# zacharie12/Hypernet-image-captioning

Hardware: AMD Instinct MI355X
Metric: training images/sec at 1/2/4/8 MI355X, Flickr30k GRU+hypernet bs=128 (higher is better)
Workload: dtype f32; 1 GPU; Flickr30k-shaped GRU+additive-attention decoder + hypernet (3 style domains), full training step (fwd, CE, bwd, clip 5.0, Adam); per_gpu_batch=128, global_batch=128, T=20, P=49, D=2048, F=200, E=200, H=200, V=9684, hypernet_params=144906720, parallelism=dp1, launch=eager, next_theta_in_adam_pass=True, next_precompute_beside_adam=True, spinup_steps=0, deterministic_gradients=True

## Files before the change

hypernet-image-captioning_amd/caphn/_lib.py:

```python
import ctypes as C
import os

import torch

_HERE = os.path.dirname(os.path.abspath(__file__))
LIB_PATH = os.environ.get("CAPHN_LIB_PATH") or os.path.join(_HERE, "libcaphn.so")
MAX_HEADS = 8

c_fp = C.c_void_p


class HyperDesc(C.Structure):
    _fields_ = [("he", C.c_int), ("n_heads", C.c_int),
                ("k", C.c_int * MAX_HEADS), ("w", C.c_int * MAX_HEADS),
                ("base_w0", c_fp), ("base_b0", c_fp), ("base_w2", c_fp), ("base_b2", c_fp),
                ("w1", c_fp * MAX_HEADS), ("b1", c_fp * MAX_HEADS),
                ("w2", c_fp * MAX_HEADS), ("b2", c_fp * MAX_HEADS),
                ("d_in", C.c_int), ("d_mid", C.c_int)]


class HyperGrads(C.Structure):
    _fields_ = [("g_base_w0", c_fp), ("g_base_b0", c_fp), ("g_base_w2", c_fp), ("g_base_b2", c_fp),
                ("g_w1", c_fp * MAX_HEADS), ("g_b1", c_fp * MAX_HEADS),
                ("g_w2", c_fp * MAX_HEADS), ("g_b2", c_fp * MAX_HEADS),
# ... 8 lines not shown

_DEC_FIELDS = ("fc0_w", "fc0_b", "fc2_w", "fc2_b", "embed_w", "out_w", "out_b", "Wa_w", "Wa_b",
               "Ua_w", "Ua_b", "va_w", "va_b", "inith_w", "inith_b", "w_ih", "w_hh", "b_ih", "b_hh",
               "initc_w", "initc_b") + tuple(f"{a}{i}" for a in ("lw_ih", "lw_hh", "lb_ih", "lb_hh") for i in range(3))


class DecoderParams(C.Structure):
    _fields_ = [(n, c_fp) for n in _DEC_FIELDS]


class DecoderGrads(C.Structure):
    _fields_ = [(n, c_fp) for n in _DEC_FIELDS]


class AdamHParams(C.Structure):
    _fields_ = [("lr", C.c_float), ("beta1", C.c_float), ("beta2", C.c_float), ("eps", C.c_float),
                ("step", C.c_int), ("dev_scalars", c_fp), ("zero_gfac", C.c_int)]


class RankJob(C.Structure):
    _fields_ = [("W", c_fp), ("m", c_fp), ("v", c_fp), ("gfac", c_fp), ("ldg", C.c_size_t), ("afac", c_fp), ("lda", C.c_size_t),
                ("next_a", c_fp), ("next_bias", c_fp), ("next_theta", c_fp), ("rows", C.c_int), ("k", C.c_int),
                ("next_pack", c_fp), ("pack_H", C.c_int), ("pack_HA", C.c_int), ("pack_pitch", C.c_int), ("pack_hrows", C.c_int)]


class PairPack(C.Structure):
    _fields_ = [("wp", c_fp), ("H", C.c_int), ("HA", C.c_int), ("pitch", C.c_int), ("hrows", C.c_int)]


MAX_LAYERS = 4


class PlainDims(C.Structure):
    _fields_ = [(n, C.c_int) for n in ("B", "T", "E", "H", "V", "L", "cell")]


class AttnDims(C.Structure):
    _fields_ = [(n, C.c_int) for n in ("bs", "nh", "dh", "tq", "tk", "q_ldt", "q_ldb", "k_ldt", "k_ldb", "v_ldt", "v_ldb",
                                       "o_ldt", "o_ldb")] + [("scale", C.c_float), ("dropout_p", C.c_float),
                                                             ("seed", C.c_uint64)]


class PlainParams(C.Structure):
    _fields_ = [("embed_w", c_fp), ("out_w", c_fp), ("out_b", c_fp),
                ("w_ih", c_fp * MAX_LAYERS), ("w_hh", c_fp * MAX_LAYERS), ("b_ih", c_fp * MAX_LAYERS), ("b_hh", c_fp * MAX_LAYERS)]


class PlainGrads(C.Structure):
    _fields_ = [("embed_w", c_fp), ("out_w", c_fp), ("out_b", c_fp),
                ("w_ih", c_fp * MAX_LAYERS), ("w_hh", c_fp * MAX_LAYERS), ("b_ih", c_fp * MAX_LAYERS), ("b_hh", c_fp * MAX_LAYERS),
                ("features", c_fp)]


class SearchCfg(C.Structure):
    _fields_ = [("n_images", C.c_int), ("beam", C.c_int), ("max_steps", C.c_int), ("zero_pad_rule", C.c_int),
                ("lookup_first", C.c_int), ("first_token", C.c_int64), ("end_token", C.c_int64)]


SIGNATURES = {
    "caphn_abi_version": (C.c_int, []),
    "caphn_device_arch": (C.c_int, [C.c_char_p, C.c_int]),
    "caphn_device_error": (C.c_int, [C.c_int]),
    "caphn_gemm_f32": (C.c_int, [C.c_int, C.c_int, C.c_int, C.c_int, C.c_int, c_fp, C.c_int, c_fp, C.c_int,
                                 c_fp, C.c_int, c_fp, c_fp, C.c_int, C.c_int, C.c_int, c_fp]),
    "caphn_split3_bf16": (C.c_int, [c_fp, C.c_int, C.c_int, C.c_int, c_fp, C.c_int, C.c_size_t, C.c_int, c_fp]),
    "caphn_gemm_planes_f32": (C.c_int, [C.c_int, C.c_int, C.c_int, C.c_int, C.c_int, c_fp, C.c_int, c_fp, C.c_int, C.c_size_t,
                                        c_fp, C.c_int, c_fp, C.c_int, C.c_size_t, c_fp, C.c_int, c_fp, c_fp, C.c_int, C.c_int,
                                        C.c_int, C.c_int, c_fp]),
    "caphn_zero_f32": (C.c_int, [c_fp, C.c_size_t, c_fp]),
    "caphn_lrelu_bwd_f32": (C.c_int, [C.c_size_t, c_fp, c_fp, c_fp, c_fp]),
    "caphn_axpy_f32": (C.c_int, [C.c_size_t, C.c_float, c_fp, c_fp, c_fp]),
    "caphn_scale_f32": (C.c_int, [C.c_size_t, c_fp, c_fp, c_fp, c_fp]),
    "caphn_add_dropout_f32": (C.c_int, [C.c_size_t, c_fp, c_fp, C.c_float, C.c_uint64, C.c_uint64, c_fp, c_fp]),
    "caphn_dropout_f32": (C.c_int, [C.c_size_t, C.c_float, C.c_uint64, C.c_uint64, c_fp, c_fp, c_fp]),
    "caphn_colsum_workspace_bytes": (C.c_size_t, [C.c_int, C.c_int]),
    "caphn_linear_wgrad_f32": (C.c_int, [C.c_int, C.c_int, C.c_int, c_fp, C.c_int, c_fp, C.c_int, c_fp, C.c_int, c_fp, c_fp, c_fp]),
    "caphn_colsum_f32": (C.c_int, [C.c_int, C.c_int, c_fp, C.c_int, c_fp, c_fp, c_fp]),
    "caphn_hyper_acts_floats": (C.c_int, [C.POINTER(HyperDesc)]),
    "caphn_hyper_forward": (C.c_int, [C.POINTER(HyperDesc), c_fp, c_fp, c_fp, c_fp]),
    "caphn_hyper_backward_workspace_bytes": (C.c_size_t, [C.POINTER(HyperDesc)]),
    "caphn_hyper_backward": (C.c_int, [C.POINTER(HyperDesc), c_fp, c_fp, C.POINTER(HyperGrads), c_fp, c_fp]),
    "caphn_decoder_workspace_bytes": (C.c_size_t, [C.POINTER(DecoderDims)]),
    "caphn_decoder_forward": (C.c_int, [C.POINTER(DecoderDims), C.POINTER(DecoderParams), c_fp, c_fp,
                                        c_fp, c_fp, c_fp, c_fp]),
    "caphn_decoder_pair_prep": (C.c_int, [C.POINTER(DecoderDims), C.POINTER(DecoderParams), c_fp, c_fp]),
    "caphn_decoder_pair_pack_desc": (C.c_int, [C.POINTER(DecoderDims), c_fp, C.POINTER(PairPack)]),
    "caphn_decoder_precompute": (C.c_int, [C.POINTER(DecoderDims), C.POINTER(DecoderParams), c_fp, c_fp, c_fp, c_fp]),
    "caphn_decoder_inputs": (C.c_int, [C.POINTER(DecoderDims), C.POINTER(DecoderParams), c_fp, c_fp, c_fp]),
    "caphn_decoder_lookup": (C.c_int, [C.POINTER(DecoderDims), C.POINTER(DecoderParams), c_fp, c_fp, c_fp]),
    "caphn_decoder_prepare_rows": (C.c_int, [C.POINTER(DecoderDims), c_fp, C.c_int64, c_fp, c_fp]),
    "caphn_decoder_forward_sampled": (C.c_int, [C.POINTER(DecoderDims), C.POINTER(DecoderParams), c_fp, c_fp,
# ... 123 lines not shown
```

hypernet-image-captioning_amd/csrc/decoder.hip:

```cpp
#include "common.h"
#include "decoder_internal.h"
#include "gemm_internal.h"
#include <algorithm>
#include <initializer_list>
#include <mutex>

int g_tune_deterministic = 0;
int g_tune_rec_pair = 1;
int g_tune_rec_rotate = 1;
int g_tune_vocab_order = 1;
int g_tune_branch_mask = 7;
int g_tune_splitk_target = 1280;
int g_tune_chain_main = 0;
int g_tune_hops = 0;
int g_tune_fork = 4;
int g_tune_join_chain = 0;
int g_tune_sk_dhs = 0, g_tune_sk_vocab_w = 0;
#define RUN(x) do { int _rc = (x); if (_rc != CAPHN_OK) return _rc; } while (0)

namespace {

struct Side {
    hipStream_t st[3];
    enum { D_FORK = 0, D_JOIN = 1, D_X = 4, D_MS = 10, D_PRE_F = 14, D_PRE_ALL = 15, D_COUNT = 16 };
    struct Dep { hipEvent_t ev; unsigned seq = 0; bool by_value = false; };
    Dep deps[D_COUNT];
    unsigned* vals = nullptr;
    unsigned counter = 0;
    bool values = false;
    bool pre_valid = false;
    const void* pre_ws = nullptr;
    bool ready = false, on = false;
    bool forked[3] = {false, false, false};
    hipStream_t main = nullptr;
    int init() {
        if (ready) return CAPHN_OK;
        static std::mutex mu;
        std::lock_guard<std::mutex> lock(mu);
        if (ready) return CAPHN_OK;
        for (auto& s : st) if (hipStreamCreateWithFlags(&s, hipStreamNonBlocking) != hipSuccess) return CAPHN_ELAUNCH;
// ... 626 lines not shown
    a.drop_p = d->dropout_p; a.drop_seed = d->dropout_seed;
    const int ang = w.L1 > 0 ? 0 : pair ? caphn_rec_pair_bwd_groups(P, H) : caphn_rec_bwd_groups(P, H);
    if (ang > 0) { a.dWaf = ws + w.dWaf; a.apart = ws + w.apart; }
    if (w.L1 > 0) {
        RUN(caphn_zero_f32(ws + w.dcarry, (size_t)B * H, s));
        a.dHs = ws + w.dH0; a.dh0 = ws + w.dcarry; a.drop_p = 0.f;
        for (int t = T - 1; t >= 0; --t) {
            RUN(layers_backward(d, p, w, ws, t + 1, ws + w.dHs + (size_t)t * H, T * H, ws + w.dcarry, ws + w.dH0 + (size_t)t * H, T * H, s));
            a.t0 = t; a.t1 = t + 1;
            RUN(caphn_launch_rec_bwd(a, lstm, s));
        }
        RUN(layers_backward(d, p, w, ws, 0, ws + w.dcarry, H, nullptr, ws + w.dh0, H, s));
    } else if (pair) {
        a.xch = reinterpret_cast<unsigned long long*>(ws + w.xch) + w.xch_floats * sizeof(float) / sizeof(unsigned long long);
        a.apart_rows = ang;
        a.WP = ws + w.wp; a.wp_pitch = caphn_rec_pair_pitch(H);
        if (!raw) { a.inith_w = p->inith_w; a.initc_w = lstm ? p->initc_w : nullptr; a.dmean_part = ws + w.dmeanf; a.F = F; }
        RUN(caphn_launch_rec_pair_bwd(a, lstm, s));
    } else
    RUN(caphn_launch_rec_bwd(a, lstm, s));

    hipStream_t b0 = sd.s(0), b1 = sd.s(1), b2 = sd.s(2);
    const bool t_main = hook != nullptr && g_tune_chain_main != 0;
    hipStream_t sT = t_main ? s : b1, sF = t_main ? b1 : s;
    const bool hold_big = late && !raw && fork_mode == 3;
    RUN(sd.fork_many({0, 1, 2}));
    if (late && !hold_big) {
        RUN(wgrad_bias(V, H, BT, dlogits, LV, ws + w.Hs, H, g->out_w, H, g->out_b, rmap, cws, b0, gz));
        RUN(sd.milestone(CAPHN_MS_VOCAB, b0));
    }
    if (ctx_side) RUN(sd.wait(5, sT));
    else if (!(d->precomputed & 32)) RUN(caphn_launch_ctx(B, T, P, F, ws + w.alphas, f, ws + w.ctx, EF, sT));
    if (lstm) RUN(gemm_auto(1, 0, GH, EF, BT, dgi, GH, ws + w.Xe, EF, g->w_ih, EF, nullptr, 0, sT, nullptr, 0, gz));
    else RUN(wgrad_bias(GH, EF, BT, dgi, GH, ws + w.Xe, EF, g->w_ih, EF, g->b_ih, nullptr, cw1, sT, gz));
    RUN(wgrad_bias(GH, H, BT, dgh, GH, ws + w.Hprev, H, g->w_hh, H, g->b_hh, nullptr, cw2, b2, gz));
    if (lstm) RUN(caphn_colsum_f32(BT, GH, dgi, GH, g->b_ih, cw2, b2));
    RUN(sd.record(3, b2));
    hipStream_t se = late ? b2 : b0;
    RUN(caphn_gemm_f32(0, 0, BT, E, GH, dgi, GH, p->w_ih, EF, ws + w.dXe, E, nullptr, nullptr, 0, 0, 1, se));
    if (!gz) RUN(caphn_zero_f32(g->embed_w, (size_t)V * E, se));
    RUN(caphn_embedding_scatter_add_v(BT, E, V, ws + w.dXe, idx, g->embed_w, se));
    RUN(sd.milestone(CAPHN_MS_EMBED, se));
    RUN(sd.wait(3, sT));
    RUN(sd.milestone(CAPHN_MS_DTHETA, sT));
    if (hook && !hold_big) {
        RUN(caphn_hyper_backward(hook->hd, g->w_ih, hook->acts, hook->hg, hook->ws, sT));
// ... 292 lines not shown
```

hypernet-image-captioning_amd/csrc/gemm_bf16x3.hip:

```cpp
#include "common.h"
#include "gemm_internal.h"
#include "split3.h"
#include <type_traits>

#ifdef CAPHN_GEMM_PROFILE
__device__ unsigned long long d_gemm_prof[10];
__device__ unsigned long long d_gemm_wgt[2 * 8192];
extern "C" int caphn_debug_gemm_wgtimes(unsigned long long* out, int n) {
    return hipMemcpyFromSymbol(out, HIP_SYMBOL(d_gemm_wgt), sizeof(unsigned long long) * 2 * (n < 8192 ? n : 8192)) == hipSuccess ? 0 : -1;
}
#define GSTAMP(i) do { if (gprof) { unsigned long long _n = clock64(); gpc[i] += _n - glast; glast = _n; } } while (0)
extern "C" int caphn_debug_gemm_prof(unsigned long long* out, int reset) {
    if (out && hipMemcpyFromSymbol(out, HIP_SYMBOL(d_gemm_prof), sizeof(unsigned long long) * 10) != hipSuccess) return -1;
    if (reset) { unsigned long long z[10] = {0, 0, 0, 0, 0, 0, 0, 0, 0, 0}; if (hipMemcpyToSymbol(HIP_SYMBOL(d_gemm_prof), z, sizeof(z)) != hipSuccess) return -1; }
    return 0;
}
#else
#define GSTAMP(i) do { } while (0)
#endif

extern int g_tune_gemm_waves;
namespace {

constexpr int BK = 32;
// ... 186 lines not shown
                *reinterpret_cast<bf16x8*>(p + pl * PLANE) = v;
            }
        }
    }
    __device__ static __forceinline__ bf16x8 frag(const __bf16* __restrict__ S, int plane, int row0, int ks, int lane) {
        if (KC) {
            return *reinterpret_cast<const bf16x8*>(S + plane * PLANE + kc_off(row0 + (lane & 31), ks * 16 + (lane >> 5) * 8));
        } else {
            const int g = lane >> 4, i = lane & 15;
            const int col = row0 + 16 * (g & 1) + 4 * (i & 3);
            const int kb = 16 * ks + 8 * (g >> 1) + (i >> 2);
            typedef __attribute__((address_space(3))) bf16x4 lds_bf16x4;
            const __bf16* p = S + plane * PLANE + kb * PITCHM + col;
            const bf16x4 lo4 = __builtin_amdgcn_ds_read_tr16_b64_v4bf16((lds_bf16x4*)(p));
            const bf16x4 hi4 = __builtin_amdgcn_ds_read_tr16_b64_v4bf16((lds_bf16x4*)(p + 4 * PITCHM));
            return __builtin_shufflevector(lo4, hi4, 0, 1, 2, 3, 4, 5, 6, 7);
        }
    }
};

__device__ __forceinline__ float bf16_bits_to_f32(unsigned short b) { return __uint_as_float((unsigned)b << 16); }

template <int BM, int BN, bool TA, bool TB, int MODE>
__device__ __forceinline__ void gemm_bf16x3_body(GemmArgs g) {
    constexpr bool PL = MODE == 1;
    constexpr bool SINGLE = MODE == 2;
    constexpr bool WS = MODE == 5;
    constexpr bool DB = MODE == 3 || WS;
    constexpr bool TWO = MODE == 4;
    using TileA = TileS<BM, !TA>;
    using TileB = TileS<BN, TB>;
    constexpr int WM = BM / 2, WN = BN / 2, TM = WM / 32, TN = WN / 32;
    constexpr int TILE_ELEMS = TileA::ELEMS + TileB::ELEMS;
    extern __shared__ __attribute__((aligned(16))) __bf16 lds[];
    __bf16* As = lds;
    __bf16* Bs = lds + TileA::ELEMS;
    __bf16* As1 = DB ? lds + TILE_ELEMS : As;
    __bf16* Bs1 = DB ? lds + TILE_ELEMS + TileA::ELEMS : Bs;

    const bool producer = WS && threadIdx.x >= 256;
    const int tid = WS ? (threadIdx.x & 255) : threadIdx.x, lane = tid & 63, wave = tid >> 6;
    const int wm = wave >> 1, wn = wave & 1;
    const int li = lane & 31, kh = lane >> 5;
#ifdef CAPHN_GEMM_PROFILE
    const unsigned long long gstart = clock64();
    const unsigned gwg = blockIdx.x + gridDim.x * (blockIdx.y + gridDim.y * blockIdx.z);
    if (tid == 0 && gwg < 8192) d_gemm_wgt[2 * gwg] = wall_clock64();
#endif
    int bx = blockIdx.x, by = blockIdx.y, bz = blockIdx.z;
    if (g.flags & (1 << 20)) {
        const int nx = gridDim.x, ny = gridDim.y, nwg = nx * ny * (int)gridDim.z;
        const int orig = bx + nx * (by + ny * bz);
        const int xcd = orig & 7, q = nwg >> 3, r = nwg & 7;
        const int wgid = (xcd < r ? xcd * (q + 1) : r * (q + 1) + (xcd - r) * q) + (orig >> 3);
        if (g.flags & (1 << 22)) { by = wgid % ny; bx = (wgid / ny) % nx; }
        else { bx = wgid % nx; by = (wgid / nx) % ny; }
        bz = wgid / (nx * ny);
    }
    const int m0 = by * BM, n0 = bx * BN;
    const int* rmapA = nullptr; const int* kmap = nullptr;
    if (g.map_mode == 1) { g.M = min(g.M, g.dev_count[0]); rmapA = g.row_map; if (m0 >= g.M) return; }
    if (g.map_mode == 2) { g.K = min(g.K, g.dev_count[0]); kmap = g.row_map; }

    const int nslab_total = (g.K + BK - 1) / BK;
    int slab0 = 0, slab1 = nslab_total;
    if (g.splitk > 1) {
        const int sps = g.map_mode == 2 ? (nslab_total + g.splitk - 1) / g.splitk : g.slabs_per_split;
        slab0 = bz * sps;
        slab1 = min(nslab_total, slab0 + sps);
        if (slab0 >= slab1) return;
    }

    constexpr bool DUAL = TM * TN == 1;
    f32x16 acc[TM][TN], acc2[DUAL ? TM : 1][DUAL ? TN : 1];
#pragma unroll
    for (int a = 0; a < TM; ++a)
#pragma unroll
        for (int b = 0; b < TN; ++b)
#pragma unroll
            for (int r = 0; r < 16; ++r) { acc[a][b][r] = 0.f; if (DUAL) acc2[a][b][r] = 0.f; }

    f32x4 ra0[TileA::NV], rb0[TileB::NV], ra1[TileA::NV], rb1[TileB::NV];
    int pra[TileA::NV], prb[TileB::NV];
    const int* kl = nullptr;
    const int kbase = slab0 * BK;
    bool fast = !(g.flags & (1 << 21)) && g.vecA && g.vecB && g.M >= 4 && g.N >= 4 && g.K >= 4 && (g.K & 3) == 0 &&
                (!TA || (g.M & 3) == 0) && (TB || (g.N & 3) == 0);
    if (kmap) {
        const int need = (slab1 - slab0) * BK;
        if (fast && TA && !TB && g.kmap_lds >= need) {
            int* kls = reinterpret_cast<int*>(lds + (DB ? 2 : 1) * TILE_ELEMS);
            for (int i = tid; i < need; i += 256) kls[i] = kmap[min(kbase + i, g.K - 1)];
// ... 353 lines not shown
            for (int r = 0; r < 16; ++r) {
                const int row = m0 + wm * WM + a * 32 + (r & 3) + 8 * (r >> 2) + 4 * kh;
                if (row >= g.M) continue;
                float v = acc[a][b][r] + bv;
                float* c = g.C + (size_t)(rmapA ? rmapA[row] : row) * g.ldc + col;
                if (atomic) { atomicAdd(c, v); continue; }
                if (g.flags & CAPHN_GEMM_ACCUM) v += *c;
                if (g.flags & CAPHN_GEMM_RELU) v = fmaxf(v, 0.f);
                if (g.flags & CAPHN_GEMM_LRELU) v = v > 0.f ? v : 0.01f * v;
                if (g.flags & CAPHN_GEMM_MASK) v = (g.mask[(size_t)row * g.ldmask + col] > 0.f) ? v : 0.f;
                *c = v;
            }
        }
#ifdef CAPHN_GEMM_PROFILE
    if (tid == 0) {
        __builtin_amdgcn_s_waitcnt(0);
        if (gwg < 8192) d_gemm_wgt[2 * gwg + 1] = wall_clock64();
        if (gwg == 0) atomicAdd(&d_gemm_prof[8], clock64() - gstart);
    }
#endif
}

template <int BM, int BN, bool TA, bool TB, int MODE>
__global__ __launch_bounds__(256) void gemm_bf16x3_kernel(GemmArgs g) { gemm_bf16x3_body<BM, BN, TA, TB, MODE>(g); }
template <int BM, int BN, bool TA, bool TB, int MODE>
__global__ __launch_bounds__(256) __attribute__((amdgpu_waves_per_eu(5, 5))) void gemm_bf16x3_kernel_w5(GemmArgs g) { gemm_bf16x3_body<BM, BN, TA, TB, MODE>(g); }
template <int BM, int BN, bool TA, bool TB, int MODE>
__global__ __launch_bounds__(256) __attribute__((amdgpu_waves_per_eu(6, 6))) void gemm_bf16x3_kernel_w6(GemmArgs g) { gemm_bf16x3_body<BM, BN, TA, TB, MODE>(g); }

template <int BM, int BN, bool TA, bool TB>
__global__ __launch_bounds__(512) void gemm_bf16x3_kernel_ws(GemmArgs g) { gemm_bf16x3_body<BM, BN, TA, TB, 5>(g); }

template <int BM, int BN, bool TA, bool TB, int PL>
int launch_one(const GemmArgs& g, hipStream_t s) {
    using TileA = TileS<BM, !TA>;
    using TileB = TileS<BN, TB>;
    constexpr size_t lds_tiles = sizeof(__bf16) * (TileA::ELEMS + TileB::ELEMS) * ((PL == 3 || PL == 5) ? 2 : 1);
    size_t lds = lds_tiles;
    if (g.kmap_lds > 0) lds += sizeof(int) * (size_t)g.kmap_lds;
    static bool attr_set[64];
    int dev = 0;
    if (hipGetDevice(&dev) != hipSuccess || dev < 0 || dev >= 64) return CAPHN_ELAUNCH;
    if (lds_tiles + 16384 > 48 * 1024 && !attr_set[dev]) {
        const void* fn = PL == 5 ? reinterpret_cast<const void*>(gemm_bf16x3_kernel_ws<BM, BN, TA, TB>)
                                 : reinterpret_cast<const void*>(gemm_bf16x3_kernel<BM, BN, TA, TB, PL == 5 ? 0 : PL>);
        if (hipFuncSetAttribute(fn, hipFuncAttributeMaxDynamicSharedMemorySize, (int)(lds_tiles + 16384)) != hipSuccess) return CAPHN_ELAUNCH;
        attr_set[dev] = true;
    }
    dim3 grid((g.N + BN - 1) / BN, (g.M + BM - 1) / BM, g.splitk > 1 ? g.splitk : 1);
    if constexpr (PL == 5) {
        hipLaunchKernelGGL((gemm_bf16x3_kernel_ws<BM, BN, TA, TB>), grid, dim3(512), lds, s, g);
        return caphn_launch_status();
    } else {
    if constexpr (BM == 64 && PL == 0) {
// ... 28 lines not shown
    bool pl = g_tune_gemm_planes && g.Ap && g.Bp && !(ta && tb) && (g.K % 8) == 0 && g.K >= 8 && (g.ldap % 8) == 0 && (g.ldbp % 8) == 0 &&
              (g.psa % 8) == 0 && (g.psb % 8) == 0 && caphn_aligned16(g.Ap) && caphn_aligned16(g.Bp);
    if (pl && ta && (((g.M + 7) & ~7) > g.ldap || g.M < 8)) pl = false;
    if (pl && !tb && (((g.N + 7) & ~7) > g.ldbp || g.N < 8)) pl = false;
    if (pl && g.map_mode == 2) {
        const int nslab = (g.K + 31) / 32, sk = g.splitk > 1 ? g.splitk : 1;
        if (!(ta && !tb) || ((nslab + sk - 1) / sk) * 32 > 4096) pl = false;
    }
    return pl;
}
template <int BM, int BN, bool TA, bool TB>
static int occ_one() {
    using TileA = TileS<BM, !TA>;
    using TileB = TileS<BN, TB>;
    int n = 0;
    if (hipOccupancyMaxActiveBlocksPerMultiprocessor(&n, reinterpret_cast<const void*>(gemm_bf16x3_kernel<BM, BN, TA, TB, 0>), 256,
                                                     sizeof(__bf16) * (TileA::ELEMS + TileB::ELEMS)) != hipSuccess) return -1;
    return n;
}
extern "C" int caphn_debug_gemm_occupancy(int ta, int tb, int tile) {
    if (tile == 128) return !ta && tb ? occ_one<128, 128, false, true>() : !ta ? occ_one<128, 128, false, false>() : !tb ? occ_one<128, 128, true, false>() : occ_one<128, 128, true, true>();
    return !ta && tb ? occ_one<64, 64, false, true>() : !ta ? occ_one<64, 64, false, false>() : !tb ? occ_one<64, 64, true, false>() : occ_one<64, 64, true, true>();
}
int caphn_gemm_bf16x3_launch(GemmArgs g, int ta, int tb, hipStream_t s) {
    if (g_tune_gemm_xcd) g.flags |= 1 << 20;
    g.kmap_lds = 0;
    if (g.map_mode == 2 && ta && !tb) {
        const int nslab = (g.K + 31) / 32, sk = g.splitk > 1 ? g.splitk : 1;
        const int ints = ((nslab + sk - 1) / sk) * 32;
        if (ints <= 4096) g.kmap_lds = ints;
    }
    if (!g_tune_gemm_fast) g.flags |= 1 << 21;
    {
        const double ea = ta ? (double)g.K * g.lda : (double)g.M * g.lda, eb = tb ? (double)g.N * g.ldb : (double)g.K * g.ldb;
        if (ea * 4.0 >= 4.0e9 || eb * 4.0 >= 4.0e9) g.flags |= 1 << 21;
    }
    if (g_tune_gemm_order != 0 && g.splitk <= 1) {
        const double abytes = 4.0 * (double)g.M * g.K, bbytes = 4.0 * (double)g.N * g.K, l2 = 3.0 * 1024 * 1024;
        if (g_tune_gemm_order == 2 || (bbytes > l2 && abytes < bbytes)) g.flags |= 1 << 22;
    }
    long tiles128 = (long)((g.M + 127) / 128) * ((g.N + 127) / 128) * g.splitk;
    if (g.K < 512) tiles128 = 0;
    if (g_tune_gemm_tile == 64) tiles128 = 0; else if (g_tune_gemm_tile == 128) tiles128 = 1 << 20;
    const bool pl = caphn_gemm_planes_ok(g, ta, tb);
    if (!pl && g_tune_gemm_single == 0 && g_tune_gemm_tile == 0 && g_tune_gemm_ws == 0) {
        const int rc = caphn_gemm_kres_launch(g, ta, tb, s);
        if (rc != 1) return rc;
    }
    if (pl) {
        if (tiles128 >= 512) return launch_cfg<128, 128, 1>(g, ta, tb, s);
        return launch_cfg<64, 64, 1>(g, ta, tb, s);
    }
    if (g_tune_gemm_single == 1 && !(ta && tb)) {
        if (tiles128 >= 512) return launch_cfg<128, 128, 2>(g, ta, tb, s);
        return launch_cfg<64, 64, 2>(g, ta, tb, s);
    }
    if (g_tune_gemm_single == 2 && !(ta && tb)) {
        if (tiles128 >= 512) return launch_cfg<128, 128, 4>(g, ta, tb, s);
        return launch_cfg<64, 64, 4>(g, ta, tb, s);
    }
    if (g_tune_gemm_ws == 128 && !(ta && tb)) return launch_cfg<128, 128, 5>(g, ta, tb, s);
    if (g_tune_gemm_ws == 64 && !(ta && tb)) return launch_cfg<64, 64, 5>(g, ta, tb, s);
    if (tiles128 >= 512) return launch_cfg<128, 128, 0>(g, ta, tb, s);
    const int lay = (!ta && tb) ? 1 : (!ta && !tb) ? 2 : (ta && !tb) ? 4 : 0;
    if (g_tune_gemm_db & lay) return launch_cfg<64, 64, 3>(g, ta, tb, s);
    return launch_cfg<64, 64, 0>(g, ta, tb, s);
}

namespace {
struct SplitJobs { SplitJob j[8]; int n; long block0[9]; };
__global__ __launch_bounds__(256) void split3_kernel(SplitJobs jobs) {
    int ji = 0;
    for (int i = 1; i < jobs.n; ++i) if ((long)blockIdx.x >= jobs.block0[i]) ji = i;
    const SplitJob& J = jobs.j[ji];
    const int cpr = (J.cols + 7) >> 3;
    const long nchunk = (long)(J.rows + J.zero_rows) * cpr;
    const long stride = (jobs.block0[ji + 1] - jobs.block0[ji]) * 256;
    __bf16* dst = static_cast<__bf16*>(J.dst);
    const bool vec = (J.ld & 3) == 0 && caphn_aligned16_dev(J.src);
    for (long c = ((long)blockIdx.x - jobs.block0[ji]) * 256 + threadIdx.x; c < nchunk; c += stride) {
        const int row = (int)(c / cpr), col = (int)(c % cpr) * 8;
        const float* sp = J.src + (size_t)row * J.ld + col;
        f32x4 v0 = {0.f, 0.f, 0.f, 0.f}, v1 = {0.f, 0.f, 0.f, 0.f};
        if (row >= J.rows) { }
        else if (vec && col + 8 <= J.cols) { v0 = *reinterpret_cast<const f32x4*>(sp); v1 = *reinterpret_cast<const f32x4*>(sp + 4); }
        else {
#pragma unroll
            for (int e = 0; e < 4; ++e) { if (col + e < J.cols) v0[e] = sp[e]; if (col + 4 + e < J.cols) v1[e] = sp[4 + e]; }
        }
// ... 29 lines not shown
```

hypernet-image-captioning_amd/csrc/gemm_internal.h:

```cpp
#pragma once
#include "common.h"

struct GemmArgs {
    int M, N, K;
    const float* A; int lda;
    const float* B; int ldb;
    float* C; int ldc;
    const float* bias;
    const float* mask; int ldmask;
    int flags;
    int splitk, slabs_per_split;
    int vecA, vecB;
    const int* row_map; const int* dev_count; int map_mode;
    float* colsum_a;
    int kmap_lds;
    const void* Ap; int ldap; size_t psa;
    const void* Bp; int ldbp; size_t psb;
};

struct Opnd {
    const float* f; int ld;
    const void* p; int ldp; size_t ps;
    Opnd() : f(nullptr), ld(0), p(nullptr), ldp(0), ps(0) {}
    Opnd(const float* f_, int ld_) : f(f_), ld(ld_), p(nullptr), ldp(0), ps(0) {}
// ... 8 lines not shown
struct GemmX {
    const float* bias = nullptr; const float* mask = nullptr; int ldmask = 0; int flags = 0; int splitk = 1;
    const int* rowmap = nullptr;
    int map_mode = 0;
    float* colsum = nullptr;
    int Kp = 0;
};
int caphn_gemm_x(int ta, int tb, int M, int N, int K, const Opnd& A, const Opnd& B, float* C, int ldc, const GemmX& x, hipStream_t s);

struct SplitJob { const float* src; int ld; void* dst; int ldp; size_t ps; int rows, cols; int zero_rows; };
int caphn_split3_launch(const SplitJob* jobs, int n, hipStream_t s);

int caphn_gemm_mapped(int ta, int tb, int M, int N, int K, const float* A, int lda, const float* B, int ldb,
                      float* C, int ldc, const float* bias, int flags, int splitk,
                      const int* row_map, const int* dev_count, int map_mode, hipStream_t s);

int caphn_gemm_tn_colsum(int M, int N, int K, const float* A, int lda, const float* B, int ldb, float* C, int ldc,
                         float* colsum_out, int splitk, const int* rowmap, void* cws, bool prezeroed, hipStream_t s);

bool caphn_gemm_planes_ok(const GemmArgs& g, int ta, int tb);
int caphn_gemm_bf16x3_launch(GemmArgs g, int ta, int tb, hipStream_t s);
int caphn_gemm_kres_launch(const GemmArgs& g, int ta, int tb, hipStream_t s);
extern int g_tune_gemm;
```

hypernet-image-captioning_amd/csrc/hyper.hip:

```cpp
#include "common.h"
#include <algorithm>

namespace {

constexpr float LRELU = 0.01f;
__device__ __forceinline__ float lrelu(float v) { return v > 0.f ? v : LRELU * v; }
__device__ __forceinline__ float lrelu_grad(float post) { return post > 0.f ? 1.f : LRELU; }

struct GemvJob {
    const float* W; const float* b; const float* x; float* y;
    int rows, k, act, vec;
    int block0, nblocks;
    float* xcopy;
};
struct GemvJobs { GemvJob j[CAPHN_MAX_HEADS]; int n; };

template <int QMAX, int RB, bool NTL>
__device__ __forceinline__ void gemv_rows_wave(const GemvJob& J, int wave_g, int nwaves, int lane) {
    const int k4 = J.k >> 2;
    const f32x4* x4 = reinterpret_cast<const f32x4*>(J.x);
    f32x4 xr[QMAX];
#pragma unroll
    for (int q = 0; q < QMAX; ++q) {
        int c = lane + 64 * q;
// ... 810 lines not shown
extern int g_tune_gemm_xcd;
extern int g_tune_gemm_fast;
extern int g_tune_gemm_planes;
extern int g_tune_rec_pair;
extern int g_tune_gemm_single;
extern int g_tune_gemm_tile;
extern int g_tune_deterministic;
extern int g_tune_adam_cap;
extern int g_tune_chain_main;
extern int g_tune_rec_cache;
extern int g_tune_splitk_target;
extern int g_tune_gemm_order;
extern int g_tune_branch_mask;
extern int g_tune_gemm_db;
extern int g_tune_gemm_ws;
extern int g_tune_adam_dense_cap;
extern int g_tune_sk_dhs, g_tune_sk_vocab_w;
extern int g_tune_join_chain;
extern int g_tune_gemm_kres;
extern int g_tune_gemm_waves;
extern int g_tune_hops;
extern int g_tune_vocab_order;
extern int g_det_vocab;
int caphn_rec_pair_debug_skip(int v);
int caphn_rec_pair_debug_opts(int v);
extern "C" int caphn_tune(int key, int value) {
    if (key == 0) { g_tune_gemv = value; return CAPHN_OK; }
    if (key == 1) { g_tune_adam = value; return CAPHN_OK; }
    if (key == 2) { g_tune_gemm = value; return CAPHN_OK; }
    if (key == 3) { g_tune_rec_rotate = value; return CAPHN_OK; }
    if (key == 4) { g_tune_fork = value; return CAPHN_OK; }
    if (key == 6) { g_tune_gemm_xcd = value; return CAPHN_OK; }
    if (key == 7) { g_tune_gemm_fast = value; return CAPHN_OK; }
    if (key == 8) { g_tune_gemm_planes = value; return CAPHN_OK; }
    if (key == 9) { g_tune_rec_pair = value; return CAPHN_OK; }
    if (key == 10) return caphn_rec_pair_debug_skip(value);
    if (key == 11) { g_tune_gemm_single = value; return CAPHN_OK; }
    if (key == 12) { g_tune_gemm_tile = value; return CAPHN_OK; }
    if (key == 13) { g_tune_deterministic = value > 0; g_det_vocab = value; return CAPHN_OK; }
    if (key == 21) { g_tune_vocab_order = value != 0; return CAPHN_OK; }
    if (key == 20) { if (value < 0 || value > 7) return CAPHN_EINVAL; g_tune_branch_mask = value; return CAPHN_OK; }
    if (key == 18) { if (value < 0 || value > 2) return CAPHN_EINVAL; g_tune_gemm_order = value; return CAPHN_OK; }
    if (key == 17) { if (value < 1 || value > 65536) return CAPHN_EINVAL; g_tune_splitk_target = value; return CAPHN_OK; }
    if (key == 16) { if (value < 0 || value > 2) return CAPHN_EINVAL; g_tune_rec_cache = value; return CAPHN_OK; }
    if (key == 15) { g_tune_chain_main = value != 0; return CAPHN_OK; }
    if (key == 26) { g_tune_hops = value != 0; return CAPHN_OK; }
    if (key == 27) { g_tune_hyper_tail = value != 0; return CAPHN_OK; }
    if (key == 28) { g_tune_acts_fused = value != 0; return CAPHN_OK; }
    if (key == 36) { g_tune_gemm_kres = value != 0; return CAPHN_OK; }
    if (key == 35) { g_tune_join_chain = value != 0; return CAPHN_OK; }
    if (key == 33) { if (value < 0 || value > 64) return CAPHN_EINVAL; g_tune_sk_dhs = value; return CAPHN_OK; }
    if (key == 34) { if (value < 0 || value > 64) return CAPHN_EINVAL; g_tune_sk_vocab_w = value; return CAPHN_OK; }
    if (key == 30) { if (value < 64 || value > 4096) return CAPHN_EINVAL; g_tune_vjp_blocks = value; return CAPHN_OK; }
    if (key == 31) { if (value < 64 || value > 65535) return CAPHN_EINVAL; g_tune_adam_dense_cap = value; return CAPHN_OK; }
    if (key == 29) { if (value != 0 && value != 64 && value != 128) return CAPHN_EINVAL; g_tune_gemm_ws = value; return CAPHN_OK; }
    if (key == 25) { if (value != 0 && value != 5 && value != 6) return CAPHN_EINVAL; g_tune_gemm_waves = value; return CAPHN_OK; }
    if (key == 24) return caphn_rec_pair_debug_opts(value);
    if (key == 23) { if (value < 0 || value > 7) return CAPHN_EINVAL; g_tune_gemm_db = value; return CAPHN_OK; }
    if (key == 22) { if (value < 1) return CAPHN_EINVAL; g_tune_xch_timeout = 100ll * value; return CAPHN_OK; }
    if (key == 14) { if (value < 64 || value > 65535) return CAPHN_EINVAL; g_tune_adam_cap = value; return CAPHN_OK; }
    return CAPHN_EINVAL;
}
```

include/caphn.h:

```cpp
#ifndef CAPHN_H
#define CAPHN_H
#include <stdint.h>
#include <stddef.h>

#ifdef __cplusplus
extern "C" {
#endif

typedef void* caphn_stream_t;

#define CAPHN_OK 0
#define CAPHN_EINVAL (-1)
#define CAPHN_ELAUNCH (-2)
#define CAPHN_ELIMIT (-3)
#define CAPHN_ETIMEOUT (-4)

int caphn_abi_version(void);
int caphn_device_error(int clear);
int caphn_device_arch(char* buf, int buflen);

#define CAPHN_GEMM_BIAS 1
#define CAPHN_GEMM_RELU 2
#define CAPHN_GEMM_ACCUM 4
#define CAPHN_GEMM_MASK 8
#define CAPHN_GEMM_LRELU 16
int caphn_gemm_f32(int ta, int tb, int M, int N, int K,
                   const float* A, int lda, const float* B, int ldb,
                   float* C, int ldc, const float* bias,
                   const float* mask, int ldmask, int flags, int splitk,
                   caphn_stream_t stream);

int caphn_split3_bf16(const float* src, int rows, int cols, int ld, void* planes, int ldp, size_t plane_stride, int zero_rows,
                      caphn_stream_t stream);
int caphn_gemm_planes_f32(int ta, int tb, int M, int N, int K,
                          const float* A, int lda, const void* Ap, int ldap, size_t psa,
                          const float* B, int ldb, const void* Bp, int ldbp, size_t psb,
                          float* C, int ldc, const float* bias, const float* mask, int ldmask, int flags, int splitk,
                          int Kp, caphn_stream_t stream);

int caphn_zero_f32(float* p, size_t n, caphn_stream_t stream);
int caphn_dropout_f32(size_t n, float p, unsigned long long seed, unsigned long long offset, const float* in, float* out,
                      caphn_stream_t stream);
int caphn_add_dropout_f32(size_t n, const float* x, const float* branch, float p, unsigned long long seed,
                          unsigned long long offset, float* out, caphn_stream_t stream);
int caphn_scale_f32(size_t n, const float* x, const float* scale_dev, float* out, caphn_stream_t stream);
int caphn_lrelu_bwd_f32(size_t n, const float* dy, const float* post, float* dx, caphn_stream_t stream);
int caphn_axpy_f32(size_t n, float alpha, const float* x, float* y, caphn_stream_t stream);
int caphn_linear_wgrad_f32(int M, int N, int K, const float* dY, int ldy, const float* X, int ldx, float* dW, int ldw,
                           float* db, void* ws, caphn_stream_t stream);
size_t caphn_colsum_workspace_bytes(int M, int N);
int caphn_colsum_f32(int M, int N, const float* A, int lda, float* out, void* ws, caphn_stream_t stream);

#define CAPHN_MAX_HEADS 8
typedef struct caphn_hyper_desc {
    int he;
    int n_heads;
    int k[CAPHN_MAX_HEADS];
    int w[CAPHN_MAX_HEADS];
    const float* base_w0; const float* base_b0;
    const float* base_w2; const float* base_b2;
    const float* w1[CAPHN_MAX_HEADS]; const float* b1[CAPHN_MAX_HEADS];
// ... 250 lines not shown
```

Baseline: 50760 images/s.

## Batch decoder backward tail weight-gradient GEMMs into one grouped kernel launch

```diff
diff --git a/hypernet-image-captioning_amd/caphn/_lib.py b/hypernet-image-captioning_amd/caphn/_lib.py
--- a/hypernet-image-captioning_amd/caphn/_lib.py
+++ b/hypernet-image-captioning_amd/caphn/_lib.py
@@ -54,6 +54,11 @@
     _fields_ = [("W", c_fp), ("m", c_fp), ("v", c_fp), ("gfac", c_fp), ("ldg", C.c_size_t), ("afac", c_fp), ("lda", C.c_size_t),
                 ("next_a", c_fp), ("next_bias", c_fp), ("next_theta", c_fp), ("rows", C.c_int), ("k", C.c_int),
                 ("next_pack", c_fp), ("pack_H", C.c_int), ("pack_HA", C.c_int), ("pack_pitch", C.c_int), ("pack_hrows", C.c_int)]
+
+
+class GemmJob(C.Structure):
+    _fields_ = [("M", C.c_int), ("N", C.c_int), ("K", C.c_int), ("A", c_fp), ("lda", C.c_int), ("B", c_fp), ("ldb", C.c_int),
+                ("C", c_fp), ("ldc", C.c_int), ("colsum", c_fp), ("rowmap", c_fp)]
 
 
 class PairPack(C.Structure):
@@ -99,6 +104,7 @@
     "caphn_gemm_planes_f32": (C.c_int, [C.c_int, C.c_int, C.c_int, C.c_int, C.c_int, c_fp, C.c_int, c_fp, C.c_int, C.c_size_t,
                                         c_fp, C.c_int, c_fp, C.c_int, C.c_size_t, c_fp, C.c_int, c_fp, c_fp, C.c_int, C.c_int,
                                         C.c_int, C.c_int, c_fp]),
+    "caphn_gemm_group_f32": (C.c_int, [C.c_int, C.c_int, C.c_int, C.POINTER(GemmJob), C.c_int, c_fp]),
     "caphn_zero_f32": (C.c_int, [c_fp, C.c_size_t, c_fp]),
     "caphn_lrelu_bwd_f32": (C.c_int, [C.c_size_t, c_fp, c_fp, c_fp, c_fp]),
     "caphn_axpy_f32": (C.c_int, [C.c_size_t, C.c_float, c_fp, c_fp, c_fp]),
diff --git a/hypernet-image-captioning_amd/csrc/decoder.hip b/hypernet-image-captioning_amd/csrc/decoder.hip
--- a/hypernet-image-captioning_amd/csrc/decoder.hip
+++ b/hypernet-image-captioning_amd/csrc/decoder.hip
@@ -16,6 +16,7 @@
 int g_tune_fork = 4;
 int g_tune_join_chain = 0;
 int g_tune_sk_dhs = 0, g_tune_sk_vocab_w = 0;
+int g_tune_tail_group = 1;
 #define RUN(x) do { int _rc = (x); if (_rc != CAPHN_OK) return _rc; } while (0)
 
 namespace {
@@ -688,6 +689,43 @@
 
     hipStream_t b0 = sd.s(0), b1 = sd.s(1), b2 = sd.s(2);
     const bool t_main = hook != nullptr && g_tune_chain_main != 0;
+    if (g_tune_tail_group && g_tune_gemm == 1 && pair && !lstm && !raw && w.L1 == 0 && ang > 0 && !late && !t_main && sd.on &&
+        g_tune_branch_mask == 7) {
+        RUN(sd.fork_many({1, 2}));
+        if (ctx_side) RUN(sd.wait(5, b1));
+        else if (!(d->precomputed & 32)) RUN(caphn_launch_ctx(B, T, P, F, ws + w.alphas, f, ws + w.ctx, EF, b1));
+        const bool det = g_tune_deterministic != 0;
+        GemmGroup tn(1, 0), nn(0, 0);
+        RUN(tn.add(GH, EF, BT, dgi, GH, ws + w.Xe, EF, g->w_ih, EF, g->b_ih, nullptr, true, gz));
+        RUN(tn.add(GH, H, BT, dgh, GH, ws + w.Hprev, H, g->w_hh, H, g->b_hh, nullptr, true, gz));
+        RUN(tn.add(H, F, BP, ws + w.dWaf, H, f, F, g->Wa_w, F, g->Wa_b, nullptr, true, gz));
+        RUN(tn.add(H, H, BT, ws + w.duah, H, ws + w.Hprev, H, g->Ua_w, H, g->Ua_b, nullptr, true, gz));
+        RUN(tn.add(H, F, B, ws + w.dh0, H, ws + w.meanf, F, g->inith_w, F, g->inith_b, nullptr, true, gz));
+        RUN(tn.launch(b1, det));
+        RUN(sd.milestone(CAPHN_MS_DTHETA, b1));
+        if (hook) RUN(caphn_hyper_backward(hook->hd, g->w_ih, hook->acts, hook->hg, hook->ws, b1));
+        RUN(sd.milestone(CAPHN_MS_HYPER, b1));
+        RUN(nn.add(BT, E, GH, dgi, GH, p->w_ih, EF, ws + w.dXe, E, nullptr, nullptr, false, false));
+        RUN(nn.add(BT, F, GH, dgi, GH, p->w_ih + E, EF, ws + w.dctx, F, nullptr, nullptr, false, false));
+        RUN(nn.launch(s, det));
+        RUN(sd.record(3, s));
+        RUN(caphn_launch_df(B, T, P, F, ws + w.alphas, ws + w.dctx, ws + w.dmeanf, ws + w.df, s, ws + w.dmeanf + (size_t)B * F));
+        RUN(caphn_gemm_f32(0, 0, BP, F, H, ws + w.dWaf, H, p->Wa_w, F, ws + w.df, F, nullptr, nullptr, 0, CAPHN_GEMM_ACCUM, 1, s));
+        RUN(sd.record(4, s));
+        RUN(caphn_gemm_f32(0, 0, BP, F, F, ws + w.df, F, p->fc2_w, F, ws + w.dY1, F, nullptr, ws + w.Y1, F, CAPHN_GEMM_MASK, 1, s));
+        RUN(wgrad_bias(F, D, BP, ws + w.dY1, F, features, D, g->fc0_w, D, g->fc0_b, nullptr, cw0, s, gz));
+        RUN(sd.wait(3, b2));
+        if (!gz) RUN(caphn_zero_f32(g->embed_w, (size_t)V * E, b2));
+        RUN(caphn_embedding_scatter_add_v(BT, E, V, ws + w.dXe, idx, g->embed_w, b2));
+        RUN(sd.milestone(CAPHN_MS_EMBED, b2));
+        RUN(caphn_colsum_f32(B * ang, H + 1, ws + w.apart, H + 1, ws + w.vtmp, cw2, b2));
+        hipLaunchKernelGGL(copy2_kernel, dim3((H + 256) / 256), dim3(256), 0, b2, ws + w.vtmp, H, g->va_w, g->va_b);
+        RUN(sd.wait(4, b2));
+        RUN(wgrad_bias(F, F, BP, ws + w.df, F, ws + w.Y1, F, g->fc2_w, F, g->fc2_b, nullptr, cw2, b2, gz));
+        if (g_tune_join_chain) { RUN(sd.join_into(0, 1)); RUN(sd.join_into(2, 1)); RUN(sd.jointo(1)); }
+        else { RUN(sd.jointo(0)); RUN(sd.jointo(1)); RUN(sd.jointo(2)); }
+        return caphn_launch_status();
+    }
     hipStream_t sT = t_main ? s : b1, sF = t_main ? b1 : s;
     const bool hold_big = late && !raw && fork_mode == 3;
     RUN(sd.fork_many({0, 1, 2}));
diff --git a/hypernet-image-captioning_amd/csrc/gemm_bf16x3.hip b/hypernet-image-captioning_amd/csrc/gemm_bf16x3.hip
--- a/hypernet-image-captioning_amd/csrc/gemm_bf16x3.hip
+++ b/hypernet-image-captioning_amd/csrc/gemm_bf16x3.hip
@@ -232,7 +232,7 @@
 __device__ __forceinline__ float bf16_bits_to_f32(unsigned short b) { return __uint_as_float((unsigned)b << 16); }
 
 template <int BM, int BN, bool TA, bool TB, int MODE>
-__device__ __forceinline__ void gemm_bf16x3_body(GemmArgs g) {
+__device__ __forceinline__ void gemm_bf16x3_body(GemmArgs g, int bx, int by, int bz, const int nx, const int ny, const int nz) {
     constexpr bool PL = MODE == 1;
     constexpr bool SINGLE = MODE == 2;
     constexpr bool WS = MODE == 5;
@@ -257,9 +257,8 @@
     const unsigned gwg = blockIdx.x + gridDim.x * (blockIdx.y + gridDim.y * blockIdx.z);
     if (tid == 0 && gwg < 8192) d_gemm_wgt[2 * gwg] = wall_clock64();
 #endif
-    int bx = blockIdx.x, by = blockIdx.y, bz = blockIdx.z;
     if (g.flags & (1 << 20)) {
-        const int nx = gridDim.x, ny = gridDim.y, nwg = nx * ny * (int)gridDim.z;
+        const int nwg = nx * ny * nz;
         const int orig = bx + nx * (by + ny * bz);
         const int xcd = orig & 7, q = nwg >> 3, r = nwg & 7;
         const int wgid = (xcd < r ? xcd * (q + 1) : r * (q + 1) + (xcd - r) * q) + (orig >> 3);
@@ -275,9 +274,12 @@
     const int nslab_total = (g.K + BK - 1) / BK;
     int slab0 = 0, slab1 = nslab_total;
     if (g.splitk > 1) {
-        const int sps = g.map_mode == 2 ? (nslab_total + g.splitk - 1) / g.splitk : g.slabs_per_split;
-        slab0 = bz * sps;
-        slab1 = min(nslab_total, slab0 + sps);
+        if (g.flags & (1 << 23)) caphn_gemm_krange(nslab_total, g.splitk, bz, slab0, slab1);
+        else {
+            const int sps = g.map_mode == 2 ? (nslab_total + g.splitk - 1) / g.splitk : g.slabs_per_split;
+            slab0 = bz * sps;
+            slab1 = min(nslab_total, slab0 + sps);
+        }
         if (slab0 >= slab1) return;
     }
 
@@ -677,14 +679,36 @@
 }
 
 template <int BM, int BN, bool TA, bool TB, int MODE>
-__global__ __launch_bounds__(256) void gemm_bf16x3_kernel(GemmArgs g) { gemm_bf16x3_body<BM, BN, TA, TB, MODE>(g); }
+__global__ __launch_bounds__(256) void gemm_bf16x3_kernel(GemmArgs g) {
+    gemm_bf16x3_body<BM, BN, TA, TB, MODE>(g, blockIdx.x, blockIdx.y, blockIdx.z, gridDim.x, gridDim.y, gridDim.z);
+}
 template <int BM, int BN, bool TA, bool TB, int MODE>
-__global__ __launch_bounds__(256) __attribute__((amdgpu_waves_per_eu(5, 5))) void gemm_bf16x3_kernel_w5(GemmArgs g) { gemm_bf16x3_body<BM, BN, TA, TB, MODE>(g); }
+__global__ __launch_bounds__(256) __attribute__((amdgpu_waves_per_eu(5, 5))) void gemm_bf16x3_kernel_w5(GemmArgs g) {
+    gemm_bf16x3_body<BM, BN, TA, TB, MODE>(g, blockIdx.x, blockIdx.y, blockIdx.z, gridDim.x, gridDim.y, gridDim.z);
+}
 template <int BM, int BN, bool TA, bool TB, int MODE>
-__global__ __launch_bounds__(256) __attribute__((amdgpu_waves_per_eu(6, 6))) void gemm_bf16x3_kernel_w6(GemmArgs g) { gemm_bf16x3_body<BM, BN, TA, TB, MODE>(g); }
+__global__ __launch_bounds__(256) __attribute__((amdgpu_waves_per_eu(6, 6))) void gemm_bf16x3_kernel_w6(GemmArgs g) {
+    gemm_bf16x3_body<BM, BN, TA, TB, MODE>(g, blockIdx.x, blockIdx.y, blockIdx.z, gridDim.x, gridDim.y, gridDim.z);
+}
 
 template <int BM, int BN, bool TA, bool TB>
-__global__ __launch_bounds__(512) void gemm_bf16x3_kernel_ws(GemmArgs g) { gemm_bf16x3_body<BM, BN, TA, TB, 5>(g); }
+__global__ __launch_bounds__(512) void gemm_bf16x3_kernel_ws(GemmArgs g) {
+    gemm_bf16x3_body<BM, BN, TA, TB, 5>(g, blockIdx.x, blockIdx.y, blockIdx.z, gridDim.x, gridDim.y, gridDim.z);
+}
+
+struct GemmGroupTable {
+    GemmArgs g[GEMM_GROUP_MAX];
+    int first[GEMM_GROUP_MAX + 1], nx[GEMM_GROUP_MAX], ny[GEMM_GROUP_MAX];
+    int n;
+};
+template <bool TA, bool TB>
+__global__ __launch_bounds__(256) void gemm_bf16x3_group_kernel(GemmGroupTable t) {
+    const int p = caphn_gemm_group_slot(t.first, t.n, (int)blockIdx.x);
+    const int local = (int)blockIdx.x - t.first[p];
+    const int nx = t.nx[p], ny = t.ny[p];
+    const GemmArgs g = t.g[p];
+    gemm_bf16x3_body<64, 64, TA, TB, 0>(g, local % nx, (local / nx) % ny, local / (nx * ny), nx, ny, g.splitk);
+}
 
 template <int BM, int BN, bool TA, bool TB, int PL>
 int launch_one(const GemmArgs& g, hipStream_t s) {
@@ -759,7 +783,7 @@
     if (tile == 128) return !ta && tb ? occ_one<128, 128, false, true>() : !ta ? occ_one<128, 128, false, false>() : !tb ? occ_one<128, 128, true, false>() : occ_one<128, 128, true, true>();
     return !ta && tb ? occ_one<64, 64, false, true>() : !ta ? occ_one<64, 64, false, false>() : !tb ? occ_one<64, 64, true, false>() : occ_one<64, 64, true, true>();
 }
-int caphn_gemm_bf16x3_launch(GemmArgs g, int ta, int tb, hipStream_t s) {
+static void prep_args(GemmArgs& g, int ta, int tb) {
     if (g_tune_gemm_xcd) g.flags |= 1 << 20;
     g.kmap_lds = 0;
     if (g.map_mode == 2 && ta && !tb) {
@@ -776,6 +800,9 @@
         const double abytes = 4.0 * (double)g.M * g.K, bbytes = 4.0 * (double)g.N * g.K, l2 = 3.0 * 1024 * 1024;
         if (g_tune_gemm_order == 2 || (bbytes > l2 && abytes < bbytes)) g.flags |= 1 << 22;
     }
+}
+int caphn_gemm_bf16x3_launch(GemmArgs g, int ta, int tb, hipStream_t s) {
+    prep_args(g, ta, tb);
     long tiles128 = (long)((g.M + 127) / 128) * ((g.N + 127) / 128) * g.splitk;
     if (g.K < 512) tiles128 = 0;
     if (g_tune_gemm_tile == 64) tiles128 = 0; else if (g_tune_gemm_tile == 128) tiles128 = 1 << 20;
@@ -802,6 +829,154 @@
     const int lay = (!ta && tb) ? 1 : (!ta && !tb) ? 2 : (ta && !tb) ? 4 : 0;
     if (g_tune_gemm_db & lay) return launch_cfg<64, 64, 3>(g, ta, tb, s);
     return launch_cfg<64, 64, 0>(g, ta, tb, s);
+}
+
+int caphn_gemm_group_plan(int n, const int* M, const int* N, const int* K, const int* splittable, int target, int min_slabs,
+                          GemmGroupPlan* out) {
+    if (n < 1 || n > GEMM_GROUP_MAX || !M || !N || !K || !out || min_slabs < 1) return CAPHN_EINVAL;
+    long tiles[GEMM_GROUP_MAX]; int nslab[GEMM_GROUP_MAX], split[GEMM_GROUP_MAX];
+    long work = 0, pinned = 0;
+    for (int i = 0; i < n; ++i) {
+        if (M[i] <= 0 || N[i] <= 0 || K[i] <= 0) return CAPHN_EINVAL;
+        tiles[i] = (long)((M[i] + 63) / 64) * ((N[i] + 63) / 64);
+        nslab[i] = (K[i] + 31) / 32;
+        const bool can = splittable && splittable[i] && nslab[i] >= 2 * min_slabs;
+        split[i] = can ? 0 : 1;
+        if (can) work += tiles[i] * nslab[i]; else pinned += tiles[i];
+    }
+    const long room = target - pinned > 1 ? target - pinned : 1;
+    long L = (work + room - 1) / room;
+    if (L < min_slabs) L = min_slabs;
+    for (int i = 0; i < n; ++i) {
+        if (split[i]) continue;
+        long sk = (nslab[i] + L - 1) / L;
+        if (sk > nslab[i] / min_slabs) sk = nslab[i] / min_slabs;
+        split[i] = sk < 1 ? 1 : (int)sk;
+    }
+    int order[GEMM_GROUP_MAX];
+    for (int i = 0; i < n; ++i) order[i] = i;
+    for (int i = 1; i < n; ++i) {
+        const int m = order[i];
+        const int len = (nslab[m] + split[m] - 1) / split[m];
+        int j = i;
+        while (j > 0 && (nslab[order[j - 1]] + split[order[j - 1]] - 1) / split[order[j - 1]] < len) { order[j] = order[j - 1]; --j; }
+        order[j] = m;
+    }
+    long first = 0;
+    out->n = n;
+    for (int i = 0; i < n; ++i) {
+        const int m = order[i];
+        out->member[i] = m; out->splitk[i] = split[m];
+        out->nx[i] = (N[m] + 63) / 64; out->ny[i] = (M[m] + 63) / 64;
+        out->first[i] = (int)first;
+        first += tiles[m] * split[m];
+        if (first > (1l << 30)) return CAPHN_ELIMIT;
+    }
+    out->first[n] = out->total = (int)first;
+    return CAPHN_OK;
+}
+extern "C" int caphn_debug_gemm_group_plan(int n, const int* M, const int* N, const int* K, const int* splittable, int target,
+                                           int min_slabs, int* head, int* items, int max_items) {
+    GemmGroupPlan pl;
+    const int rc = caphn_gemm_group_plan(n, M, N, K, splittable, target, min_slabs, &pl);
+    if (rc != CAPHN_OK || !head) return rc != CAPHN_OK ? rc : CAPHN_EINVAL;
+    head[0] = pl.total;
+    for (int i = 0; i < n; ++i) {
+        int* h = head + 1 + 5 * i;
+        h[0] = pl.member[i]; h[1] = pl.splitk[i]; h[2] = pl.nx[i]; h[3] = pl.ny[i]; h[4] = pl.first[i];
+    }
+    for (int wg = 0; items && wg < pl.total && wg < max_items; ++wg) {
+        const int p = caphn_gemm_group_slot(pl.first, pl.n, wg), local = wg - pl.first[p];
+        const int nslab = (K[pl.member[p]] + 31) / 32;
+        int s0 = 0, s1 = nslab;
+        if (pl.splitk[p] > 1) caphn_gemm_krange(nslab, pl.splitk[p], local / (pl.nx[p] * pl.ny[p]), s0, s1);
+        int* it = items + 5 * wg;
+        it[0] = pl.member[p]; it[1] = local % pl.nx[p]; it[2] = (local / pl.nx[p]) % pl.ny[p]; it[3] = s0; it[4] = s1;
+    }
+    return CAPHN_OK;
+}
+
+int GemmGroup::add(int M, int N, int K, const float* A, int lda, const float* B, int ldb, float* C, int ldc, float* colsum,
+                   const int* rowmap, bool can_split, bool prezeroed_) {
+    if (n >= GEMM_GROUP_MAX || M <= 0 || N <= 0 || K <= 0 || !A || !B || !C || (ta && tb) || (colsum && !ta) || (rowmap && !ta))
+        return CAPHN_EINVAL;
+    GemmArgs& a = g[n];
+    a.M = M; a.N = N; a.K = K; a.A = A; a.lda = lda; a.B = B; a.ldb = ldb; a.C = C; a.ldc = ldc;
+    a.bias = nullptr; a.mask = nullptr; a.ldmask = 0; a.flags = 0;
+    a.splitk = 1; a.slabs_per_split = (K + 31) / 32;
+    a.vecA = caphn_aligned16(A) && (lda % 4 == 0);
+    a.vecB = caphn_aligned16(B) && (ldb % 4 == 0);
+    a.row_map = rowmap ? rowmap + 4 : nullptr; a.dev_count = rowmap; a.map_mode = rowmap ? 2 : 0;
+    a.colsum_a = colsum; a.kmap_lds = 0;
+    a.Ap = nullptr; a.Bp = nullptr; a.ldap = a.ldbp = 0; a.psa = a.psb = 0;
+    splittable[n] = can_split ? 1 : 0;
+    prezeroed[n] = prezeroed_;
+    ++n;
+    return CAPHN_OK;
+}
+extern int g_tune_splitk_target;
+int GemmGroup::launch(hipStream_t s, bool deterministic) {
+    if (n == 0) return CAPHN_OK;
+    if (g_tune_gemm != 1) return CAPHN_EINVAL;
+    int M[GEMM_GROUP_MAX], N[GEMM_GROUP_MAX], K[GEMM_GROUP_MAX], can[GEMM_GROUP_MAX];
+    for (int i = 0; i < n; ++i) { M[i] = g[i].M; N[i] = g[i].N; K[i] = g[i].K; can[i] = deterministic ? 0 : splittable[i]; }
+    GemmGroupPlan pl;
+    int rc = caphn_gemm_group_plan(n, M, N, K, can, g_tune_splitk_target, GEMM_GROUP_MIN_SLABS, &pl);
+    if (rc != CAPHN_OK) return rc;
+    GemmGroupTable t;
+    t.n = n;
+    int kmap_lds = 0;
+    for (int i = 0; i < n; ++i) {
+        GemmArgs a = g[pl.member[i]];
+        const bool pz = prezeroed[pl.member[i]];
+        a.splitk = pl.splitk[i];
+        a.slabs_per_split = ((a.K + 31) / 32 + a.splitk - 1) / a.splitk;
+        if (a.splitk > 1) a.flags |= 1 << 23;
+        if ((a.splitk > 1 || a.map_mode == 2) && !pz) {
+            if (a.ldc == a.N) { rc = caphn_zero_f32(a.C, (size_t)a.M * a.N, s); if (rc) return rc; }
+            else if (hipMemset2DAsync(a.C, sizeof(float) * a.ldc, 0, sizeof(float) * a.N, a.M, s) != hipSuccess) return CAPHN_ELAUNCH;
+        }
+        if (a.colsum_a && !pz) { rc = caphn_zero_f32(a.colsum_a, (size_t)a.M, s); if (rc) return rc; }
+        prep_args(a, ta, tb);
+        kmap_lds = a.kmap_lds > kmap_lds ? a.kmap_lds : kmap_lds;
+        t.g[i] = a; t.first[i] = pl.first[i]; t.nx[i] = pl.nx[i]; t.ny[i] = pl.ny[i];
+    }
+    t.first[n] = pl.total;
+    if (g_tune_gemm_single || g_tune_gemm_ws || g_tune_gemm_db || g_tune_gemm_waves || g_tune_gemm_tile == 128) {
+        for (int i = 0; i < n; ++i) { rc = caphn_gemm_bf16x3_launch(t.g[i], ta, tb, s); if (rc) return rc; }
+        return CAPHN_OK;
+    }
+    auto go = [&](auto ta_c, auto tb_c) -> int {
+        constexpr bool TA = decltype(ta_c)::value, TB = decltype(tb_c)::value;
+        using TileA = TileS<64, !TA>;
+        using TileB = TileS<64, TB>;
+        constexpr size_t lds_tiles = sizeof(__bf16) * (TileA::ELEMS + TileB::ELEMS);
+        static bool attr_set[64];
+        int dev = 0;
+        if (hipGetDevice(&dev) != hipSuccess || dev < 0 || dev >= 64) return CAPHN_ELAUNCH;
+        if (lds_tiles + 16384 > 48 * 1024 && !attr_set[dev]) {
+            if (hipFuncSetAttribute(reinterpret_cast<const void*>(gemm_bf16x3_group_kernel<TA, TB>),
+                                    hipFuncAttributeMaxDynamicSharedMemorySize, (int)(lds_tiles + 16384)) != hipSuccess) return CAPHN_ELAUNCH;
+            attr_set[dev] = true;
+        }
+        hipLaunchKernelGGL((gemm_bf16x3_group_kernel<TA, TB>), dim3((unsigned)pl.total), dim3(256),
+                           lds_tiles + sizeof(int) * (size_t)kmap_lds, s, t);
+        return caphn_launch_status();
+    };
+    if (!ta && tb) return go(std::false_type{}, std::true_type{});
+    if (!ta && !tb) return go(std::false_type{}, std::false_type{});
+    return go(std::true_type{}, std::false_type{});
+}
+extern int g_tune_deterministic;
+extern "C" int caphn_gemm_group_f32(int ta, int tb, int njobs, const caphn_gemm_job* jobs, int split, caphn_stream_t stream) {
+    if (njobs < 1 || njobs > GEMM_GROUP_MAX || !jobs || (ta && tb) || g_tune_gemm != 1) return CAPHN_EINVAL;
+    GemmGroup grp(ta, tb);
+    for (int i = 0; i < njobs; ++i) {
+        const caphn_gemm_job& j = jobs[i];
+        const int rc = grp.add(j.M, j.N, j.K, j.A, j.lda, j.B, j.ldb, j.C, j.ldc, j.colsum, j.rowmap, split != 0, false);
+        if (rc != CAPHN_OK) return rc;
+    }
+    return grp.launch(static_cast<hipStream_t>(stream), split == 0 || g_tune_deterministic);
 }
 
 namespace {
diff --git a/hypernet-image-captioning_amd/csrc/gemm_internal.h b/hypernet-image-captioning_amd/csrc/gemm_internal.h
--- a/hypernet-image-captioning_amd/csrc/gemm_internal.h
+++ b/hypernet-image-captioning_amd/csrc/gemm_internal.h
@@ -54,3 +54,35 @@
 int caphn_gemm_bf16x3_launch(GemmArgs g, int ta, int tb, hipStream_t s);
 int caphn_gemm_kres_launch(const GemmArgs& g, int ta, int tb, hipStream_t s);
 extern int g_tune_gemm;
+
+constexpr int GEMM_GROUP_MAX = 16;
+constexpr int GEMM_GROUP_MIN_SLABS = 16;
+
+__host__ __device__ inline void caphn_gemm_krange(int nslab, int splitk, int bz, int& s0, int& s1) {
+    const int base = nslab / splitk, rem = nslab % splitk;
+    s0 = bz * base + (bz < rem ? bz : rem);
+    s1 = s0 + base + (bz < rem ? 1 : 0);
+}
+struct GemmGroupPlan {
+    int n, total;
+    int member[GEMM_GROUP_MAX], splitk[GEMM_GROUP_MAX], nx[GEMM_GROUP_MAX], ny[GEMM_GROUP_MAX];
+    int first[GEMM_GROUP_MAX + 1];
+};
+__host__ __device__ inline int caphn_gemm_group_slot(const int* first, int n, int wg) {
+    int p = 0;
+    for (int i = 1; i < n; ++i) if (wg >= first[i]) p = i;
+    return p;
+}
+int caphn_gemm_group_plan(int n, const int* M, const int* N, const int* K, const int* splittable, int target, int min_slabs,
+                          GemmGroupPlan* out);
+
+struct GemmGroup {
+    int ta, tb, n = 0;
+    GemmArgs g[GEMM_GROUP_MAX];
+    int splittable[GEMM_GROUP_MAX];
+    bool prezeroed[GEMM_GROUP_MAX];
+    GemmGroup(int ta_, int tb_) : ta(ta_), tb(tb_) {}
+    int add(int M, int N, int K, const float* A, int lda, const float* B, int ldb, float* C, int ldc, float* colsum,
+            const int* rowmap, bool can_split, bool prezeroed_);
+    int launch(hipStream_t s, bool deterministic);
+};
diff --git a/hypernet-image-captioning_amd/csrc/hyper.hip b/hypernet-image-captioning_amd/csrc/hyper.hip
--- a/hypernet-image-captioning_amd/csrc/hyper.hip
+++ b/hypernet-image-captioning_amd/csrc/hyper.hip
@@ -856,6 +856,7 @@
 extern int g_tune_hops;
 extern int g_tune_vocab_order;
 extern int g_det_vocab;
+extern int g_tune_tail_group;
 int caphn_rec_pair_debug_skip(int v);
 int caphn_rec_pair_debug_opts(int v);
 extern "C" int caphn_tune(int key, int value) {
@@ -882,6 +883,7 @@
     if (key == 27) { g_tune_hyper_tail = value != 0; return CAPHN_OK; }
     if (key == 28) { g_tune_acts_fused = value != 0; return CAPHN_OK; }
     if (key == 36) { g_tune_gemm_kres = value != 0; return CAPHN_OK; }
+    if (key == 37) { g_tune_tail_group = value != 0; return CAPHN_OK; }
     if (key == 35) { g_tune_join_chain = value != 0; return CAPHN_OK; }
     if (key == 33) { if (value < 0 || value > 64) return CAPHN_EINVAL; g_tune_sk_dhs = value; return CAPHN_OK; }
     if (key == 34) { if (value < 0 || value > 64) return CAPHN_EINVAL; g_tune_sk_vocab_w = value; return CAPHN_OK; }
diff --git a/include/caphn.h b/include/caphn.h
--- a/include/caphn.h
+++ b/include/caphn.h
@@ -37,6 +37,15 @@
                           const float* B, int ldb, const void* Bp, int ldbp, size_t psb,
                           float* C, int ldc, const float* bias, const float* mask, int ldmask, int flags, int splitk,
                           int Kp, caphn_stream_t stream);
+typedef struct caphn_gemm_job {
+    int M, N, K;
+    const float* A; int lda;
+    const float* B; int ldb;
+    float* C; int ldc;
+    float* colsum;
+    const int* rowmap;
+} caphn_gemm_job;
+int caphn_gemm_group_f32(int ta, int tb, int njobs, const caphn_gemm_job* jobs, int split, caphn_stream_t stream);
 
 int caphn_zero_f32(float* p, size_t n, caphn_stream_t stream);
 int caphn_dropout_f32(size_t n, float p, unsigned long long seed, unsigned long long offset, const float* in, float* out,
```

Result: slower. 49590 images/s (-2.3%).
